# ssi-research/FQSS

Measured on AMD Instinct MI355X. Metric: QAT-step samples/sec + SI-SDR, ConvTasNet 2spk 8kHz W8A8, higher is better.
Workload: dtype f32; 1 GPU; ConvTasNet 2spk 8 kHz W8A8 QAT step (cfg 2), batch 8 x 4 s per GPU, quantizing phase; global_batch=8, segment_samples=32000, parallelism=dp1, optimizer=adam lr 1e-3 + clip 5.0

## Files before the change

### fqss_amd/csrc/qgemm.hip

```cpp
#include <type_traits>

#define FQSS_USES_GRAD_ADD
#include "fqss_dev.h"

namespace fqss {

typedef float f32x16 __attribute__((ext_vector_type(16)));
typedef __bf16 bf16x8 __attribute__((ext_vector_type(8)));
typedef short s16x4 __attribute__((ext_vector_type(4)));
typedef short s16x8 __attribute__((ext_vector_type(8)));

constexpr int QBM = 128, QBN = 64, QBK = 32;
constexpr int LDK = 40;
constexpr int LDN = 96;
constexpr int LDT = 36;
constexpr int WGRAD_BLOCKS = 256;

__device__ __forceinline__ unsigned short f2bf_trunc(float f) { return (unsigned short)(__float_as_uint(f) >> 16); }
__device__ __forceinline__ float bf_trunc(float f) { return __uint_as_float(__float_as_uint(f) & 0xFFFF0000u); }

__device__ __forceinline__ void split3(float g, unsigned short& b1, unsigned short& b2, unsigned short& b3) {
    const float h1 = bf_trunc(g);
    const float r1 = g - h1;
    const float h2 = bf_trunc(r1);
// ... 544 lines not shown
        for (int ks = 0; ks < W2_TK / 16; ++ks) {
            const int kk = ks * 16 + 8 * lh;
            const bf16x8 bfr = *reinterpret_cast<const bf16x8*>(&Bs[buf][wc * 32 + lr][kk]);
            bf16x8 af[GP];
#pragma unroll
            for (int p = 0; p < GP; ++p) af[p] = *reinterpret_cast<const bf16x8*>(&As[buf][p][wr * 32 + lr][kk]);
#pragma unroll
            for (int p = GP - 1; p >= 0; --p) acc = __builtin_amdgcn_mfma_f32_32x32x16_bf16(af[p], bfr, acc, 0, 0, 0);
        }
    };

    W2Stage st[W2_RING];
#pragma unroll
    for (int i = 0; i < W2_RING; ++i) load(st[i], i);
    w2_wait<3 * (W2_RING - 1)>(st[0]);
    convert_store(st[0], 0);
    load(st[0], W2_RING);
    __syncthreads();
    const bool first_half = wave < 4;
    for (int s = 0; s < nst; s += W2_RING) {
#pragma unroll
        for (int i = 0; i < W2_RING; ++i) {
            W2Stage& nx = st[(i + 1) % W2_RING];
            if (first_half) compute((s + i) & 1);
            w2_wait<3 * (W2_RING - 1)>(nx);
            convert_store(nx, s + i + 1);
            load(nx, s + i + 1 + W2_RING);
            if (!first_half) compute((s + i) & 1);
            __syncthreads();
        }
    }
#pragma unroll
    for (int i = 0; i < W2_RING; ++i) w2_wait<0>(st[i]);

#pragma unroll
    for (int i = 0; i < 2; ++i) {
        float v = rs_part[i];
#pragma unroll
        for (int o = 8; o > 0; o >>= 1) v += __shfl_xor(v, o, 64);
        if ((tid & 15) == 0) rsum[ar + 32 * i] = v;
    }
    __syncthreads();
    const float lo = *g.qmin_x, hi = *g.qmax_x;
    const float dx = (hi - lo) / 255.0f, mnx = lo;
#pragma unroll
    for (int r = 0; r < 16; ++r) {
        const int rl = (r & 3) + 8 * (r >> 2) + 4 * lh;
        const int row = row0 + wr * 32 + rl;
        const int col = col0 + wc * 32 + lr;
        if (row < g.M && col < g.N) grad_add(&g.C[(int64_t)row * g.ldc + col], dx * acc[r] + mnx * rsum[wr * 32 + rl]);
    }
}

constexpr int WGR_MAXJOBS = 25, WGR_TEAM = 8, WGR_TEAMS = 32, WGR_SLOT_FLOATS = W2_TM * 256;
struct WJob {
    const float* A; const float* A2; const unsigned char* Bc; float* C; const float* qmin; const float* qmax;
    int64_t lda, lda2, ldb, sAb, sA2b, sBb;
    int M, M1, N, K;
    int tiles_n, ntiles, spb, nstages;
    int ubeg, tile0;
    int wide;
};
struct WGroupArgs {
    int njobs, chunk, total, slots;
    unsigned* tickets; float* slabs;
    WJob j[WGR_MAXJOBS];
};
static_assert(sizeof(WGroupArgs) <= 4096, "the job table travels in the kernel arguments");
__device__ __forceinline__ void st16_sc1(float* p, const f32x4& v) {
#ifdef FQSS_NO_STORE_NOP
    asm volatile("global_store_dwordx4 %0, %1, off sc1" : : "v"(p), "v"(v) : "memory");
#else
    asm volatile("global_store_dwordx4 %0, %1, off sc1\n\ts_nop 1" : : "v"(p), "v"(v) : "memory");
#endif
}
__device__ __forceinline__ void ld16_sc1(f32x4& d, const float* p) { asm volatile("global_load_dwordx4 %0, %1, off sc1" : "=v"(d) : "v"(p) : "memory"); }

template <int GP, bool WIDE>
__device__ __forceinline__ void wgr_segment(const WGroupArgs& ga, const WJob& J, const int tile, const int s0, const int n, const int nparts,
                                            const int part, unsigned short* As_raw, unsigned short* Bs_raw, float* rsum, unsigned* ticket_s) {
    static_assert(GP == 3, "gz goes in three exact bf16 pieces");
    constexpr int TN = WIDE ? 256 : 128, NBF = WIDE ? 2 : 1;
    typedef unsigned short (*AsT)[GP][W2_TM][W2_LD];
    typedef unsigned short (*BsT)[TN][W2_LD];
    AsT As = reinterpret_cast<AsT>(As_raw);
    BsT Bs = reinterpret_cast<BsT>(Bs_raw);
    const int tid = threadIdx.x, lane = tid & 63;
    const int wave = __builtin_amdgcn_readfirstlane(tid >> 6);
    const int wr = wave >> 2, wc = wave & 3, lr = lane & 31, lh = lane >> 5;
    const int ar = tid >> 4, ac = (tid & 15) * 4;
    const int br = tid >> 2, bc = (tid & 3) * 16;
    const bool first_half = wave < 4;
    const int row0 = (tile / J.tiles_n) * W2_TM, col0 = (tile % J.tiles_n) * TN;
    const int K = J.K, spb = J.spb, nb = J.nstages / J.spb;
    const int ka_last = (K - 1) & ~3, kb_last = (K - 1) & ~15;
    const float* Arow[2];
    int64_t asb[2];
    bool aok[2];
#pragma unroll
    for (int i = 0; i < 2; ++i) {
        const int row = row0 + ar + 32 * i;
        aok[i] = row < J.M;
        const int rc = aok[i] ? row : 0;
        Arow[i] = (rc < J.M1) ? J.A + (int64_t)rc * J.lda : J.A2 + (int64_t)(rc - J.M1) * J.lda2;
        asb[i] = (rc < J.M1) ? J.sAb : J.sA2b;
    }
    const unsigned char* Brow[NBF];
#pragma unroll
    for (int f = 0; f < NBF; ++f) Brow[f] = J.Bc + (int64_t)min(col0 + br + 128 * f, J.N - 1) * J.ldb;
    const int64_t sBb = J.sBb;
    int lb = s0 / spb, lk = (s0 - lb * spb) * W2_TK;
    int ck = lk, cr = 0;
    const float* Ap[2] = {Arow[0] + lb * asb[0], Arow[1] + lb * asb[1]};
    int64_t boff = lb * sBb;
    struct Stage { f32x4 a[2]; u32x4 b[NBF]; };
    auto load = [&](Stage& st) {
#pragma unroll
        for (int i = 0; i < 2; ++i) wg_load16(st.a[i], Ap[i] + min(lk + ac, ka_last));
#pragma unroll
        for (int f = 0; f < NBF; ++f) wg_load16(st.b[f], Brow[f] + boff + min(lk + bc, kb_last));
        lk += W2_TK;
        if (lk >= spb * W2_TK) {
            lk = 0;
            lb = min(lb + 1, nb - 1);
            Ap[0] = Arow[0] + lb * asb[0];
            Ap[1] = Arow[1] + lb * asb[1];
            boff = lb * sBb;
        }
    };
    constexpr int NLD = 2 + NBF;
    auto wait_oldest = [&](Stage& st) {
        if constexpr (WIDE) asm volatile("s_waitcnt vmcnt(%4)" : "+v"(st.a[0]), "+v"(st.a[1]), "+v"(st.b[0]), "+v"(st.b[NBF - 1]) : "n"(NLD * (W2_RING - 1)) : "memory");
        else asm volatile("s_waitcnt vmcnt(%3)" : "+v"(st.a[0]), "+v"(st.a[1]), "+v"(st.b[0]) : "n"(NLD * (W2_RING - 1)) : "memory");
    };
    auto wait_all = [&](Stage& st) {
        if constexpr (WIDE) asm volatile("s_waitcnt vmcnt(0)" : "+v"(st.a[0]), "+v"(st.a[1]), "+v"(st.b[0]), "+v"(st.b[NBF - 1]) : : "memory");
        else asm volatile("s_waitcnt vmcnt(0)" : "+v"(st.a[0]), "+v"(st.a[1]), "+v"(st.b[0]) : : "memory");
    };
    float rs_part[2] = {0.f, 0.f};
    auto convert_store = [&](Stage& st, int buf) {
        const bool live = cr < n;
        const int k = ck + ac;
#pragma unroll
        for (int i = 0; i < 2; ++i) {
            float x[4];
#pragma unroll
            for (int e = 0; e < 4; ++e) x[e] = (aok[i] && live && k + e < K) ? st.a[i][e] : 0.0f;
            rs_part[i] += (x[0] + x[1]) + (x[2] + x[3]);
            uint32_t o1[2], o2[2], o3[2];
#pragma unroll
            for (int e = 0; e < 2; ++e) {
                const float a0 = x[2 * e], a1 = x[2 * e + 1];
                const float r0 = a0 - bf_trunc(a0), r1 = a1 - bf_trunc(a1);
                o1[e] = __builtin_amdgcn_perm(__float_as_uint(a1), __float_as_uint(a0), 0x07060302u);
                const float q0 = r0 - bf_trunc(r0), q1 = r1 - bf_trunc(r1);
                o2[e] = __builtin_amdgcn_perm(__float_as_uint(r1), __float_as_uint(r0), 0x07060302u);
                o3[e] = __builtin_amdgcn_perm(__float_as_uint(q1), __float_as_uint(q0), 0x07060302u);
            }
            const int row = ar + 32 * i;
            *reinterpret_cast<uint2*>(&As[buf][0][row][ac]) = make_uint2(o1[0], o1[1]);
            *reinterpret_cast<uint2*>(&As[buf][1][row][ac]) = make_uint2(o2[0], o2[1]);
            *reinterpret_cast<uint2*>(&As[buf][2][row][ac]) = make_uint2(o3[0], o3[1]);
        }
#pragma unroll
        for (int f = 0; f < NBF; ++f) {
            uint32_t o[8];
#pragma unroll
            for (int q = 0; q < 4; ++q) {
                const uint32_t w = st.b[f][q];
                const float f0 = (float)(w & 0xFFu), f1 = (float)((w >> 8) & 0xFFu);
                const float f2 = (float)((w >> 16) & 0xFFu), f3 = (float)(w >> 24);
                o[2 * q] = __builtin_amdgcn_perm(__float_as_uint(f1), __float_as_uint(f0), 0x07060302u);
                o[2 * q + 1] = __builtin_amdgcn_perm(__float_as_uint(f3), __float_as_uint(f2), 0x07060302u);
            }
            *reinterpret_cast<uint4*>(&Bs[buf][br + 128 * f][bc]) = make_uint4(o[0], o[1], o[2], o[3]);
            *reinterpret_cast<uint4*>(&Bs[buf][br + 128 * f][bc + 8]) = make_uint4(o[4], o[5], o[6], o[7]);
        }
        ++cr;
        ck += W2_TK;
        if (ck >= spb * W2_TK) ck = 0;
    };
    f32x16 acc[NBF];
#pragma unroll
    for (int f = 0; f < NBF; ++f)
#pragma unroll
        for (int r = 0; r < 16; ++r) acc[f][r] = 0.f;
    auto compute = [&](int buf) {
#pragma unroll
        for (int ks = 0; ks < W2_TK / 16; ++ks) {
            const int kk = ks * 16 + 8 * lh;
            bf16x8 bfr[NBF];
#pragma unroll
            for (int f = 0; f < NBF; ++f) bfr[f] = *reinterpret_cast<const bf16x8*>(&Bs[buf][wc * (32 * NBF) + 32 * f + lr][kk]);
            bf16x8 af[GP];
#pragma unroll
            for (int p = 0; p < GP; ++p) af[p] = *reinterpret_cast<const bf16x8*>(&As[buf][p][wr * 32 + lr][kk]);
#pragma unroll
            for (int p = GP - 1; p >= 0; --p)
#pragma unroll
                for (int f = 0; f < NBF; ++f) acc[f] = __builtin_amdgcn_mfma_f32_32x32x16_bf16(af[p], bfr[f], acc[f], 0, 0, 0);
        }
    };
    Stage st[W2_RING];
#pragma unroll
    for (int i = 0; i < W2_RING; ++i) load(st[i]);
    wait_oldest(st[0]);
    convert_store(st[0], 0);
    load(st[0]);
    __syncthreads();
    for (int s = 0; s < n; s += W2_RING) {
#pragma unroll
        for (int i = 0; i < W2_RING; ++i) {
            Stage& nx = st[(i + 1) % W2_RING];
            if (first_half) compute(i & 1);
            wait_oldest(nx);
            convert_store(nx, (i + 1) & 1);
            load(nx);
            if (!first_half) compute(i & 1);
            __syncthreads();
        }
    }
#pragma unroll
    for (int i = 0; i < W2_RING; ++i) wait_all(st[i]);
#pragma unroll
    for (int i = 0; i < 2; ++i) {
        float v = rs_part[i];
#pragma unroll
        for (int o = 8; o > 0; o >>= 1) v += __shfl_xor(v, o, 64);
        if ((tid & 15) == 0) rsum[ar + 32 * i] = v;
    }
    __syncthreads();
    const float lo = *J.qmin, hi = *J.qmax;
    const float dx = (hi - lo) / 255.0f, mnx = lo;
    constexpr int NV = 16 * NBF;
    float v[NV];
#pragma unroll
    for (int f = 0; f < NBF; ++f)
#pragma unroll
        for (int r = 0; r < 16; ++r) v[16 * f + r] = dx * acc[f][r] + mnx * rsum[wr * 32 + (r & 3) + 8 * (r >> 2) + 4 * lh];
    bool finish = nparts == 1;
    constexpr int SLOT = W2_TM * TN;
    if (!finish) {
        float* sl = ga.slabs + ((int64_t)(J.tile0 + tile) * ga.slots + part) * WGR_SLOT_FLOATS;
#pragma unroll
        for (int q = 0; q < NV / 4; ++q) st16_sc1(sl + ((int64_t)q * 512 + tid) * 4, f32x4{v[4 * q], v[4 * q + 1], v[4 * q + 2], v[4 * q + 3]});
        asm volatile("s_waitcnt vmcnt(0)" ::: "memory");
        __syncthreads();
        if (tid == 0) *ticket_s = __hip_atomic_fetch_add(&ga.tickets[J.tile0 + tile], 1u, __ATOMIC_RELAXED, __HIP_MEMORY_SCOPE_AGENT);
        __syncthreads();
        finish = *ticket_s == (unsigned)(nparts - 1);
        if (finish) {
            const float* s0p = ga.slabs + (int64_t)(J.tile0 + tile) * ga.slots * WGR_SLOT_FLOATS;
#pragma unroll
            for (int r = 0; r < NV; ++r) v[r] = 0.0f;
            for (int p = 0; p < nparts; ++p) {
#pragma unroll
                for (int h = 0; h < NBF; ++h) {
                    f32x4 t[4];
#pragma unroll
                    for (int q = 0; q < 4; ++q) ld16_sc1(t[q], s0p + (int64_t)p * WGR_SLOT_FLOATS + ((int64_t)(4 * h + q) * 512 + tid) * 4);
                    asm volatile("s_waitcnt vmcnt(0)" : "+v"(t[0]), "+v"(t[1]), "+v"(t[2]), "+v"(t[3]) : : "memory");
#pragma unroll
                    for (int q = 0; q < 4; ++q)
#pragma unroll
                        for (int e = 0; e < 4; ++e) v[16 * h + 4 * q + e] += t[q][e];
                }
            }
            if (tid == 0) __hip_atomic_store(&ga.tickets[J.tile0 + tile], 0u, __ATOMIC_RELAXED, __HIP_MEMORY_SCOPE_AGENT);
        }
    }
    static_assert(SLOT <= WGR_SLOT_FLOATS, "slab slots are sized for the wide tile");
    if (finish) {
        const int Mr = J.M, Nc = J.N;
        float* const Cp = J.C;
        float old[NV];
#pragma unroll
        for (int f = 0; f < NBF; ++f)
#pragma unroll
            for (int r = 0; r < 16; ++r) {
                const int row = row0 + wr * 32 + (r & 3) + 8 * (r >> 2) + 4 * lh, col = col0 + wc * (32 * NBF) + 32 * f + lr;
                old[16 * f + r] = (row < Mr && col < Nc) ? Cp[(int64_t)row * Nc + col] : 0.0f;
            }
#pragma unroll
        for (int f = 0; f < NBF; ++f)
#pragma unroll
            for (int r = 0; r < 16; ++r) {
                const int row = row0 + wr * 32 + (r & 3) + 8 * (r >> 2) + 4 * lh, col = col0 + wc * (32 * NBF) + 32 * f + lr;
                if (row < Mr && col < Nc) Cp[(int64_t)row * Nc + col] = old[16 * f + r] + v[16 * f + r];
            }
        asm volatile("s_waitcnt vmcnt(0)" ::: "memory");
    }
    __syncthreads();
}

template <int GP>
__global__ __launch_bounds__(512, 1) void k_qwgrad_group(WGroupArgs ga) {
    static_assert(GP == 3, "gz goes in three exact bf16 pieces");
    __shared__ __attribute__((aligned(16))) unsigned short As_raw[2 * GP * W2_TM * W2_LD];
    __shared__ __attribute__((aligned(16))) unsigned short Bs_raw[2 * 256 * W2_LD];
    __shared__ float rsum[W2_TM];
    __shared__ unsigned ticket_s;
    const int L = blockIdx.x, xcd = L % kXcds, slot = L / kXcds;
    const int team = (slot / WGR_TEAM) * kXcds + xcd, member = slot % WGR_TEAM;
    int u0 = team * ga.chunk;
    const int u1 = min(ga.total, u0 + ga.chunk);
    while (u0 < u1) {
        int jn = 0;
        for (int q = 1; q < ga.njobs; ++q) jn = (ga.j[q].ubeg <= u0) ? q : jn;
        const WJob& J = ga.j[jn];
        const int rel = u0 - J.ubeg, grp = rel / J.nstages, s0 = rel - grp * J.nstages;
        const int n = min(J.nstages - s0, u1 - u0);
        const int g0 = J.ubeg + grp * J.nstages;
        const int t_first = g0 / ga.chunk, nparts = (g0 + J.nstages - 1) / ga.chunk - t_first + 1, part = team - t_first;
        u0 += n;
        const int tile = grp * WGR_TEAM + member;
        if (tile >= J.ntiles) continue;
        if (J.wide) wgr_segment<GP, true>(ga, J, tile, s0, n, nparts, part, As_raw, Bs_raw, rsum, &ticket_s);
        else wgr_segment<GP, false>(ga, J, tile, s0, n, nparts, part, As_raw, Bs_raw, rsum, &ticket_s);
    }
}

__global__ __launch_bounds__(256) void k_wq_codes(const float* __restrict__ w, signed char* __restrict__ idx,
                                                   signed char* __restrict__ idxT, float* dw, float* rw, int Co, int Ci,
                                                   const float* __restrict__ qmin, const float* __restrict__ qmax, int n_bits) {
    __shared__ float red[4];
    const int co = blockIdx.x;
    const float L = wq_levels(n_bits), qlo = wq_qlo(n_bits), qhi = wq_qhi(n_bits);
    const float a = fmaxf(fabsf(qmin[co]), fabsf(qmax[co]));
    const float delta = (2.0f * a) / L;
    float s = 0.0f;
    for (int ci = threadIdx.x; ci < Ci; ci += 256) {
        const float X = rintf(w[(int64_t)co * Ci + ci] / delta);
        const float q = fminf(fmaxf(X, qlo), qhi);
        idx[(int64_t)co * Ci + ci] = (signed char)q;
        idxT[(int64_t)ci * Co + co] = (signed char)q;
        s += q;
    }
    float v[1] = {s};
    block_sum<float, 1>(v, red);
    if (threadIdx.x == 0) {
        dw[co] = delta;
        rw[co] = v[0];
    }
}

}

using namespace fqss;

extern "C" int fqss_wq_codes_bits(const float* w, int8_t* idx, int8_t* idxT, float* dw, float* rw, int Co, int Ci,
                                  const float* qmin, const float* qmax, int n_bits, fqss_stream_t stream) {
    FQSS_REQUIRE(w && idx && idxT && dw && rw && qmin && qmax && Co > 0 && Ci > 0, "bad args");
    FQSS_REQUIRE(n_bits >= FQSS_WQ_MIN_BITS && n_bits <= FQSS_WQ_MAX_BITS, "weight width outside 2..8 bits");
    hipLaunchKernelGGL(k_wq_codes, dim3((unsigned)Co), dim3(256), 0, (hipStream_t)stream, w, (signed char*)idx,
                       (signed char*)idxT, dw, rw, Co, Ci, qmin, qmax, n_bits);
    return launch_status("fqss_wq_codes_bits");
}

extern "C" int fqss_wq_codes(const float* w, int8_t* idx, int8_t* idxT, float* dw, float* rw, int Co, int Ci,
                             const float* qmin, const float* qmax, fqss_stream_t stream) {
    return fqss_wq_codes_bits(w, idx, idxT, dw, rw, Co, Ci, qmin, qmax, 8, stream);
}

struct QpwQuant {
    int act; const float* slope; const float *min1, *max1, *min2, *max2; uint8_t *yc1, *yc2; int64_t ld1, ld2;
    long long* stats;
    const FqssAddAfter *add1, *add2;
};

static int qpw_fwd_impl(const char* who, const uint8_t* xc, const int8_t* wi, const float* dw, const float* rw, const float* bias1,
                        const float* bias2, const float* qmin_x, const float* qmax_x, float* z1, float* z2, int B, int Ci, int Co1,
// ... 136 lines not shown

static int qpw_bwd_w_impl(const char* who, const float* gz1, const float* gz2, const uint8_t* xc, const float* qmin_x,
                          const float* qmax_x, float* gw, int B, int Ci, int Co1, int Co2, int M, int64_t ld_gz1, int64_t ld_gz2,
                          int64_t ld_xc, fqss_stream_t stream) {
    if (B == 0 || M == 0) return FQSS_OK;
    const int Co = Co1 + Co2;
    FQSS_REQUIRE(gz1 && xc && qmin_x && qmax_x && gw && (Co2 == 0 || gz2), "null tensor");
    FQSS_REQUIRE(B >= 0 && Ci > 0 && Co1 > 0 && Co2 >= 0 && M >= 0 && ld_gz1 >= M && ld_xc >= M, "bad shape");
    FQSS_REQUIRE(ld_gz1 % 4 == 0 && ld_xc % 16 == 0 && aligned16(gz1) && aligned16(xc) && ld_gz1 >= ((M + 3) & ~3),
                 "q-GEMM wgrad needs 16-B aligned gradient and code rows");
    FQSS_REQUIRE(Co2 == 0 || (ld_gz2 % 4 == 0 && aligned16(gz2) && ld_gz2 >= ((M + 3) & ~3)), "second gradient: 16-B aligned rows");
    if (B == 0 || M == 0) return FQSS_OK;
    QGemmArgs g{};
    g.A = gz1; g.B = xc; g.C = gw; g.M = Co; g.N = Ci; g.K = M;
    g.lda = ld_gz1; g.ldb = ld_xc; g.ldc = Ci;
    g.sAb = (int64_t)Co1 * ld_gz1; g.sBb = (int64_t)Ci * ld_xc; g.sCb = 0;
    g.M1 = Co1; g.A2 = gz2; g.lda2 = ld_gz2; g.sA2b = (int64_t)Co2 * ld_gz2; g.K1 = M;
    g.qmin_x = qmin_x; g.qmax_x = qmax_x;
    const int64_t tiles = cdiv(Co, 64) * cdiv(Ci, 128) * B;
    int want = (int)((WGRAD_BLOCKS + tiles / 2) / tiles);
    if (want < 1) want = 1;
    g.tiles_n = (int)cdiv(Ci, 128); g.tiles_m = (int)cdiv(Co, 64); g.batches = B;
    const int kchunk = (int)cdiv(cdiv(M, want), W2_RING * W2_TK) * W2_RING * W2_TK;
    g.kchunk = kchunk;
    g.ksplit = (int)cdiv(M, kchunk);
    hipLaunchKernelGGL(k_qwgrad2<3>, dim3(xcd_grid((int64_t)B * g.ksplit, (int64_t)g.tiles_m * g.tiles_n)), dim3(512), 0, (hipStream_t)stream, g);
    return launch_status(who);
}

extern "C" int fqss_qpw_bwd_w(const float* gz, const uint8_t* xc, const float* qmin_x, const float* qmax_x, float* gw,
                              int B, int Ci, int Co, int M, int64_t ld_gz, int64_t ld_xc, fqss_stream_t stream) {
    return qpw_bwd_w_impl("fqss_qpw_bwd_w", gz, nullptr, xc, qmin_x, qmax_x, gw, B, Ci, Co, 0, M, ld_gz, 0, ld_xc, stream);
}

extern "C" int fqss_qpw_bwd_w2(const float* gz1, const float* gz2, const uint8_t* xc, const float* qmin_x, const float* qmax_x,
                               float* gw, int B, int Ci, int Co1, int Co2, int M, int64_t ld_gz1, int64_t ld_gz2, int64_t ld_xc,
                               fqss_stream_t stream) {
    FQSS_REQUIRE(Co2 > 0, "second layer missing");
    return qpw_bwd_w_impl("fqss_qpw_bwd_w2", gz1, gz2, xc, qmin_x, qmax_x, gw, B, Ci, Co1, Co2, M, ld_gz1, ld_gz2, ld_xc, stream);
}

constexpr int64_t WGR_TICKET_BYTES = 65536;
static int wgr_plan(const FqssWgradJob* jobs, int n0, int n, WGroupArgs& ga, int64_t& slab_bytes) {
    int u = 0, t = 0, max_st = 0;
    ga.njobs = n;
    for (int q = 0; q < n; ++q) {
        const FqssWgradJob& f = jobs[n0 + q];
        WJob& J = ga.j[q];
        const int Co = f.Co1 + f.Co2;
        J.A = f.gz1; J.A2 = f.gz2; J.Bc = f.xc; J.C = f.gw; J.qmin = f.qmin_x; J.qmax = f.qmax_x;
        J.lda = f.ld_gz1; J.lda2 = f.ld_gz2; J.ldb = f.ld_xc;
        J.sAb = (int64_t)f.Co1 * f.ld_gz1; J.sA2b = (int64_t)f.Co2 * f.ld_gz2; J.sBb = (int64_t)f.Ci * f.ld_xc;
        J.M = Co; J.M1 = f.Co1; J.N = f.Ci; J.K = f.M;
        J.wide = f.Ci >= 256;
        J.tiles_n = (int)cdiv(f.Ci, J.wide ? 256 : W2_TN);
        J.ntiles = (int)cdiv(Co, W2_TM) * J.tiles_n;
        J.spb = (int)cdiv(f.M, W2_TK);
        J.nstages = f.B * J.spb;
        J.ubeg = u; J.tile0 = t;
        u += (int)cdiv(J.ntiles, WGR_TEAM) * J.nstages;
        t += J.ntiles;
        if (J.nstages > max_st) max_st = J.nstages;
    }
    ga.total = u;
    ga.chunk = (int)cdiv(u, WGR_TEAMS);
    ga.slots = (max_st - 1) / ga.chunk + 2;
    slab_bytes = (int64_t)t * ga.slots * WGR_SLOT_FLOATS * 4;
    return t;
}
static int wgr_check(const FqssWgradJob* jobs, int njobs) {
    FQSS_REQUIRE(jobs && njobs > 0, "no jobs");
    for (int q = 0; q < njobs; ++q) {
        const FqssWgradJob& f = jobs[q];
        FQSS_REQUIRE(f.gz1 && f.xc && f.qmin_x && f.qmax_x && f.gw && (f.Co2 == 0 || f.gz2), "null tensor");
        FQSS_REQUIRE(f.B > 0 && f.Ci > 0 && f.Co1 > 0 && f.Co2 >= 0 && f.M > 0 && f.ld_gz1 >= f.M && f.ld_xc >= f.M, "bad shape");
        FQSS_REQUIRE(f.ld_gz1 % 4 == 0 && f.ld_xc % 16 == 0 && aligned16(f.gz1) && aligned16(f.xc) && f.ld_gz1 >= ((f.M + 3) & ~3),
                     "q-GEMM wgrad needs 16-B aligned gradient and code rows");
        FQSS_REQUIRE(f.Co2 == 0 || (f.ld_gz2 % 4 == 0 && aligned16(f.gz2) && f.ld_gz2 >= ((f.M + 3) & ~3)), "second gradient: 16-B aligned rows");
        FQSS_REQUIRE((int64_t)f.B * cdiv(f.M, W2_TK) * cdiv(cdiv(f.Co1 + f.Co2, W2_TM) * cdiv(f.Ci, W2_TN), WGR_TEAM) < (1ll << 26), "job too large");
        for (int p = 0; p < q; ++p) FQSS_REQUIRE(jobs[p].gw != f.gw, "two jobs of one call accumulate into the same gw (plain read-modify-write)");
    }
    return FQSS_OK;
}

extern "C" int64_t fqss_qpw_bwd_w_group_ws(const FqssWgradJob* jobs, int njobs) {
    if (wgr_check(jobs, njobs) != FQSS_OK) return -1;
    int64_t need = 0;
    const int per = (int)cdiv(njobs, cdiv(njobs, WGR_MAXJOBS));
    for (int n0 = 0; n0 < njobs; n0 += per) {
        WGroupArgs ga{};
        int64_t sb = 0;
        const int t = wgr_plan(jobs, n0, njobs - n0 < per ? njobs - n0 : per, ga, sb);
        if ((int64_t)t * 4 > WGR_TICKET_BYTES) { set_error("fqss_qpw_bwd_w_group_ws: more than 16384 tiles in one launch"); return -1; }
        if (sb > need) need = sb;
    }
    return WGR_TICKET_BYTES + need;
}

extern "C" int fqss_qpw_bwd_w_group(const FqssWgradJob* jobs, int njobs, void* ws, int64_t ws_bytes, fqss_stream_t stream) {
    if (njobs == 0) return FQSS_OK;
    if (int rc = wgr_check(jobs, njobs)) return rc;
    FQSS_REQUIRE(ws && aligned16(ws), "workspace: 16-B aligned device memory (fqss_qpw_bwd_w_group_ws bytes, zero-filled when first used)");
    const int per = (int)cdiv(njobs, cdiv(njobs, WGR_MAXJOBS));
    for (int n0 = 0; n0 < njobs; n0 += per) {
        WGroupArgs ga{};
        int64_t sb = 0;
        const int t = wgr_plan(jobs, n0, njobs - n0 < per ? njobs - n0 : per, ga, sb);
        FQSS_REQUIRE((int64_t)t * 4 <= WGR_TICKET_BYTES && WGR_TICKET_BYTES + sb <= ws_bytes, "workspace too small (fqss_qpw_bwd_w_group_ws)");
        ga.tickets = (unsigned*)ws;
        ga.slabs = (float*)((char*)ws + WGR_TICKET_BYTES);
        hipLaunchKernelGGL(k_qwgrad_group<3>, dim3(WGR_TEAMS * WGR_TEAM), dim3(512), 0, (hipStream_t)stream, ga);
        if (int rc = launch_status("fqss_qpw_bwd_w_group")) return rc;
    }
    return FQSS_OK;
}

static int pwconv_fwd_x3_impl(const char* who, bool six, const float* x, const float* w, const float* bias, float* z, int B, int Ci, int Co,
                              int M, int64_t ld_x, int64_t ld_z, fqss_stream_t stream) {
    if (B == 0 || M == 0) return FQSS_OK;
    FQSS_REQUIRE(x && w && z, "null tensor");
    FQSS_REQUIRE(B >= 0 && Ci > 0 && Co > 0 && M >= 0 && ld_x >= M && ld_z >= M, "bad shape");
    FQSS_REQUIRE(Ci % 4 == 0 && ld_x % 4 == 0 && aligned16(x) && aligned16(w) && ld_x >= ((M + 3) & ~3),
                 "x3 GEMM needs Ci % 4 == 0 and 16-B aligned activation rows");
    FQSS_REQUIRE(aligned16(z) && ld_z % 4 == 0, "output rows must be 16-B aligned");
    if (B == 0 || M == 0) return FQSS_OK;
    QGemmArgs g{};
    g.A = w; g.B = x; g.C = z; g.M = Co; g.N = M; g.K = Ci;
    g.lda = Ci; g.ldb = ld_x; g.ldc = ld_z;
    g.sAb = 0; g.sBb = (int64_t)Ci * ld_x; g.sCb = (int64_t)Co * ld_z;
    g.bias = bias; g.ksplit = 1; g.kchunk = Ci; g.M1 = Co; g.K1 = Ci;
    g.tiles_n = (int)cdiv(M, QBN); g.tiles_m = (int)cdiv(Co, QBM); g.batches = B;
    if (six) hipLaunchKernelGGL((k_qgemm<3, 2>), dim3(xcd_grid((int64_t)g.tiles_n * B, g.tiles_m)), dim3(256), 0, (hipStream_t)stream, g);
    else hipLaunchKernelGGL((k_qgemm<3>), dim3(xcd_grid((int64_t)g.tiles_n * B, g.tiles_m)), dim3(256), 0, (hipStream_t)stream, g);
    return launch_status(who);
}

extern "C" int fqss_pwconv_fwd_wq(const float* x, const int8_t* wi, const float* dw, const float* bias, float* z, int B, int Ci, int Co, int M,
                                  int64_t ld_x, int64_t ld_z, fqss_stream_t stream) {
    if (B == 0 || M == 0) return FQSS_OK;
    FQSS_REQUIRE(x && wi && dw && z, "null tensor");
    FQSS_REQUIRE(B >= 0 && Ci >= 16 && Co > 0 && M >= 0 && ld_x >= M && ld_z >= M, "bad shape");
    FQSS_REQUIRE(Ci % 16 == 0 && ld_x % 4 == 0 && aligned16(x) && aligned16(wi) && ld_x >= ((M + 3) & ~3),
                 "coded-weight forward needs Ci % 16 == 0 and 16-B aligned activation rows");
    FQSS_REQUIRE(aligned16(z) && ld_z % 4 == 0, "output rows must be 16-B aligned");
    QGemmArgs g{};
    g.A = wi; g.B = x; g.C = z; g.M = Co; g.N = M; g.K = Ci;
    g.lda = Ci; g.ldb = ld_x; g.ldc = ld_z;
    g.sAb = 0; g.sBb = (int64_t)Ci * ld_x; g.sCb = (int64_t)Co * ld_z;
    g.dw = dw; g.bias = bias; g.ksplit = 1; g.kchunk = Ci; g.M1 = Co; g.K1 = Ci;
    g.B2 = x; g.ldb2 = ld_x; g.sB2b = g.sBb;
    g.tiles_n = (int)cdiv(M, QBN); g.tiles_m = (int)cdiv(Co, QBM); g.batches = B;
    hipLaunchKernelGGL((k_qgemm<4>), dim3(xcd_grid((int64_t)g.tiles_n * B, g.tiles_m)), dim3(256), 0, (hipStream_t)stream, g);
    return launch_status("fqss_pwconv_fwd_wq");
}

static int conv2_impl(const char* who, int mode, const void* A, const float* Bsig, const float* dw, const float* bias, float* C, int B, int Cr, int M,
                      int taps, int kw, int base, int row_step, int col_step, int64_t N, int64_t plane_in, int64_t plane_out,
                      fqss_stream_t stream) {
    if (B == 0 || N == 0) return FQSS_OK;
    FQSS_REQUIRE(A && Bsig && C && (mode == 3 || dw), "null tensor");
    FQSS_REQUIRE(B > 0 && Cr > 0 && M > 0 && taps >= 1 && kw >= 1 && taps % kw == 0 && N > 0 && plane_out >= N, "bad shape");
    const int64_t K = (int64_t)Cr * taps;
    FQSS_REQUIRE(K < (1 << 16), "reduction too long for the reciprocal division of the implicit loader");
    FQSS_REQUIRE(mode == 3 ? (K % 4 == 0) : (K % 16 == 0), "implicit convolution: (channels x taps) % 16 == 0 for coded weights, % 4 == 0 for float ones");
// ... 55 lines not shown
```

Baseline: 631.3 samples/s.

## Restructure grouped q-wgrad kernel: gradient fragments in registers, 256-thread blocks, 128x128 tiles

The grouped weight-gradient kernel drops the LDS staging of the three-way bf16 split of the gradient. Each wave now loads its own 32 gradient rows straight into registers and splits them into MFMA fragments. Blocks shrink from 512 to 256 threads with two blocks per CU, and each covers a fixed 128x128 tile, replacing the wide/narrow variants. Team sizes change to 4 members by 128 teams, and the code-operand conversion is pipelined one stage ahead. The intent is to cut LDS traffic and the barrier-driven convert step and to raise occupancy, at the cost of much higher register pressure (64 accumulators plus 8 f32x4 loads per stage in a 2-deep ring).

```diff
diff --git a/fqss_amd/csrc/qgemm.hip b/fqss_amd/csrc/qgemm.hip
--- a/fqss_amd/csrc/qgemm.hip
+++ b/fqss_amd/csrc/qgemm.hip
@@ -620,14 +620,13 @@
     }
 }
 
-constexpr int WGR_MAXJOBS = 25, WGR_TEAM = 8, WGR_TEAMS = 32, WGR_SLOT_FLOATS = W2_TM * 256;
+constexpr int WGR_MAXJOBS = 25, WGR_TEAM = 4, WGR_TEAMS = 128, WGR_TM = 128, WGR_TN = 128, WGR_RING = 2, WGR_SLOT_FLOATS = WGR_TM * WGR_TN;
 struct WJob {
     const float* A; const float* A2; const unsigned char* Bc; float* C; const float* qmin; const float* qmax;
     int64_t lda, lda2, ldb, sAb, sA2b, sBb;
     int M, M1, N, K;
     int tiles_n, ntiles, spb, nstages;
     int ubeg, tile0;
-    int wide;
 };
 struct WGroupArgs {
     int njobs, chunk, total, slots;
@@ -643,175 +642,185 @@
 #endif
 }
 __device__ __forceinline__ void ld16_sc1(f32x4& d, const float* p) { asm volatile("global_load_dwordx4 %0, %1, off sc1" : "=v"(d) : "v"(p) : "memory"); }
-
-template <int GP, bool WIDE>
+template <int OFF>
+__device__ __forceinline__ void wg_load16_at(f32x4& d, const void* p) {
+    asm volatile("global_load_dwordx4 %0, %1, off offset:%2" : "=v"(d) : "v"(p), "n"(OFF) : "memory");
+}
+
+struct WgrStage {
+    f32x4 a[8];
+    u32x4 b[2];
+};
+constexpr int WGR_NLD = 10;
+template <int N>
+__device__ __forceinline__ void wgr_wait(WgrStage& st) {
+    asm volatile("s_waitcnt vmcnt(%10)"
+                 : "+v"(st.a[0]), "+v"(st.a[1]), "+v"(st.a[2]), "+v"(st.a[3]), "+v"(st.a[4]), "+v"(st.a[5]), "+v"(st.a[6]), "+v"(st.a[7]),
+                   "+v"(st.b[0]), "+v"(st.b[1])
+                 : "n"(N) : "memory");
+}
+
+template <int GP>
 __device__ __forceinline__ void wgr_segment(const WGroupArgs& ga, const WJob& J, const int tile, const int s0, const int n, const int nparts,
-                                            const int part, unsigned short* As_raw, unsigned short* Bs_raw, float* rsum, unsigned* ticket_s) {
+                                            const int part, unsigned short* Bs_raw, float* rsum, unsigned* ticket_s) {
     static_assert(GP == 3, "gz goes in three exact bf16 pieces");
-    constexpr int TN = WIDE ? 256 : 128, NBF = WIDE ? 2 : 1;
-    typedef unsigned short (*AsT)[GP][W2_TM][W2_LD];
-    typedef unsigned short (*BsT)[TN][W2_LD];
-    AsT As = reinterpret_cast<AsT>(As_raw);
+    typedef unsigned short (*BsT)[WGR_TN][W2_LD];
     BsT Bs = reinterpret_cast<BsT>(Bs_raw);
     const int tid = threadIdx.x, lane = tid & 63;
     const int wave = __builtin_amdgcn_readfirstlane(tid >> 6);
-    const int wr = wave >> 2, wc = wave & 3, lr = lane & 31, lh = lane >> 5;
-    const int ar = tid >> 4, ac = (tid & 15) * 4;
+    const int lr = lane & 31, lh = lane >> 5, ao = 8 * lh;
     const int br = tid >> 2, bc = (tid & 3) * 16;
-    const bool first_half = wave < 4;
-    const int row0 = (tile / J.tiles_n) * W2_TM, col0 = (tile % J.tiles_n) * TN;
+    const int row0 = (tile / J.tiles_n) * WGR_TM, col0 = (tile % J.tiles_n) * WGR_TN;
     const int K = J.K, spb = J.spb, nb = J.nstages / J.spb;
     const int ka_last = (K - 1) & ~3, kb_last = (K - 1) & ~15;
-    const float* Arow[2];
-    int64_t asb[2];
-    bool aok[2];
-#pragma unroll
-    for (int i = 0; i < 2; ++i) {
-        const int row = row0 + ar + 32 * i;
-        aok[i] = row < J.M;
-        const int rc = aok[i] ? row : 0;
-        Arow[i] = (rc < J.M1) ? J.A + (int64_t)rc * J.lda : J.A2 + (int64_t)(rc - J.M1) * J.lda2;
-        asb[i] = (rc < J.M1) ? J.sAb : J.sA2b;
-    }
-    const unsigned char* Brow[NBF];
-#pragma unroll
-    for (int f = 0; f < NBF; ++f) Brow[f] = J.Bc + (int64_t)min(col0 + br + 128 * f, J.N - 1) * J.ldb;
+    const int row = row0 + wave * 32 + lr;
+    const int rc = row < J.M ? row : 0;
+    const bool second = rc >= J.M1;
+    const float* const Arow = second ? J.A2 + (int64_t)(rc - J.M1) * J.lda2 : J.A + (int64_t)rc * J.lda;
+    const int64_t asb = second ? J.sA2b : J.sAb;
+    const unsigned char* Brow[2];
+#pragma unroll
+    for (int f = 0; f < 2; ++f) Brow[f] = J.Bc + (int64_t)min(col0 + br + 64 * f, J.N - 1) * J.ldb;
     const int64_t sBb = J.sBb;
-    int lb = s0 / spb, lk = (s0 - lb * spb) * W2_TK;
-    int ck = lk, cr = 0;
-    const float* Ap[2] = {Arow[0] + lb * asb[0], Arow[1] + lb * asb[1]};
-    int64_t boff = lb * sBb;
-    struct Stage { f32x4 a[2]; u32x4 b[NBF]; };
-    auto load = [&](Stage& st) {
-#pragma unroll
-        for (int i = 0; i < 2; ++i) wg_load16(st.a[i], Ap[i] + min(lk + ac, ka_last));
-#pragma unroll
-        for (int f = 0; f < NBF; ++f) wg_load16(st.b[f], Brow[f] + boff + min(lk + bc, kb_last));
-        lk += W2_TK;
-        if (lk >= spb * W2_TK) {
-            lk = 0;
-            lb = min(lb + 1, nb - 1);
-            Ap[0] = Arow[0] + lb * asb[0];
-            Ap[1] = Arow[1] + lb * asb[1];
-            boff = lb * sBb;
-        }
-    };
-    constexpr int NLD = 2 + NBF;
-    auto wait_oldest = [&](Stage& st) {
-        if constexpr (WIDE) asm volatile("s_waitcnt vmcnt(%4)" : "+v"(st.a[0]), "+v"(st.a[1]), "+v"(st.b[0]), "+v"(st.b[NBF - 1]) : "n"(NLD * (W2_RING - 1)) : "memory");
-        else asm volatile("s_waitcnt vmcnt(%3)" : "+v"(st.a[0]), "+v"(st.a[1]), "+v"(st.b[0]) : "n"(NLD * (W2_RING - 1)) : "memory");
-    };
-    auto wait_all = [&](Stage& st) {
-        if constexpr (WIDE) asm volatile("s_waitcnt vmcnt(0)" : "+v"(st.a[0]), "+v"(st.a[1]), "+v"(st.b[0]), "+v"(st.b[NBF - 1]) : : "memory");
-        else asm volatile("s_waitcnt vmcnt(0)" : "+v"(st.a[0]), "+v"(st.a[1]), "+v"(st.b[0]) : : "memory");
-    };
-    float rs_part[2] = {0.f, 0.f};
-    auto convert_store = [&](Stage& st, int buf) {
-        const bool live = cr < n;
-        const int k = ck + ac;
-#pragma unroll
-        for (int i = 0; i < 2; ++i) {
-            float x[4];
-#pragma unroll
-            for (int e = 0; e < 4; ++e) x[e] = (aok[i] && live && k + e < K) ? st.a[i][e] : 0.0f;
-            rs_part[i] += (x[0] + x[1]) + (x[2] + x[3]);
-            uint32_t o1[2], o2[2], o3[2];
-#pragma unroll
-            for (int e = 0; e < 2; ++e) {
-                const float a0 = x[2 * e], a1 = x[2 * e + 1];
-                const float r0 = a0 - bf_trunc(a0), r1 = a1 - bf_trunc(a1);
-                o1[e] = __builtin_amdgcn_perm(__float_as_uint(a1), __float_as_uint(a0), 0x07060302u);
-                const float q0 = r0 - bf_trunc(r0), q1 = r1 - bf_trunc(r1);
-                o2[e] = __builtin_amdgcn_perm(__float_as_uint(r1), __float_as_uint(r0), 0x07060302u);
-                o3[e] = __builtin_amdgcn_perm(__float_as_uint(q1), __float_as_uint(q0), 0x07060302u);
-            }
-            const int row = ar + 32 * i;
-            *reinterpret_cast<uint2*>(&As[buf][0][row][ac]) = make_uint2(o1[0], o1[1]);
-            *reinterpret_cast<uint2*>(&As[buf][1][row][ac]) = make_uint2(o2[0], o2[1]);
-            *reinterpret_cast<uint2*>(&As[buf][2][row][ac]) = make_uint2(o3[0], o3[1]);
-        }
-#pragma unroll
-        for (int f = 0; f < NBF; ++f) {
+    int gb = s0 / spb, gk = (s0 - gb * spb) * W2_TK;
+    int qb = gb, qk = gk;
+    int pk = gk;
+    auto advance = [&](int& b, int& k) {
+        k += W2_TK;
+        if (k >= spb * W2_TK) { k = 0; b = min(b + 1, nb - 1); }
+    };
+    auto load_codes = [&](u32x4 (&b)[2]) {
+        const int64_t off = qb * sBb + min(qk + bc, kb_last);
+#pragma unroll
+        for (int f = 0; f < 2; ++f) wg_load16(b[f], Brow[f] + off);
+        advance(qb, qk);
+    };
+    auto load_gz = [&](f32x4 (&a)[8]) {
+        const float* const p = Arow + gb * asb;
+        if (gk + W2_TK <= K) {
+            const float* const q = p + gk + ao;
+            wg_load16_at<0>(a[0], q);   wg_load16_at<16>(a[1], q);
+            wg_load16_at<64>(a[2], q);  wg_load16_at<80>(a[3], q);
+            wg_load16_at<128>(a[4], q); wg_load16_at<144>(a[5], q);
+            wg_load16_at<192>(a[6], q); wg_load16_at<208>(a[7], q);
+        } else {
+#pragma unroll
+            for (int j = 0; j < 8; ++j) wg_load16(a[j], p + min(gk + (j >> 1) * 16 + ao + 4 * (j & 1), ka_last));
+        }
+        advance(gb, gk);
+    };
+    auto load = [&](WgrStage& st) {
+        load_gz(st.a);
+        load_codes(st.b);
+    };
+    auto convert = [&](const u32x4 (&b)[2], int buf) {
+#pragma unroll
+        for (int f = 0; f < 2; ++f) {
             uint32_t o[8];
 #pragma unroll
             for (int q = 0; q < 4; ++q) {
-                const uint32_t w = st.b[f][q];
+                const uint32_t w = b[f][q];
                 const float f0 = (float)(w & 0xFFu), f1 = (float)((w >> 8) & 0xFFu);
                 const float f2 = (float)((w >> 16) & 0xFFu), f3 = (float)(w >> 24);
                 o[2 * q] = __builtin_amdgcn_perm(__float_as_uint(f1), __float_as_uint(f0), 0x07060302u);
                 o[2 * q + 1] = __builtin_amdgcn_perm(__float_as_uint(f3), __float_as_uint(f2), 0x07060302u);
             }
-            *reinterpret_cast<uint4*>(&Bs[buf][br + 128 * f][bc]) = make_uint4(o[0], o[1], o[2], o[3]);
-            *reinterpret_cast<uint4*>(&Bs[buf][br + 128 * f][bc + 8]) = make_uint4(o[4], o[5], o[6], o[7]);
-        }
-        ++cr;
-        ck += W2_TK;
-        if (ck >= spb * W2_TK) ck = 0;
-    };
-    f32x16 acc[NBF];
-#pragma unroll
-    for (int f = 0; f < NBF; ++f)
+            *reinterpret_cast<uint4*>(&Bs[buf][br + 64 * f][bc]) = make_uint4(o[0], o[1], o[2], o[3]);
+            *reinterpret_cast<uint4*>(&Bs[buf][br + 64 * f][bc + 8]) = make_uint4(o[4], o[5], o[6], o[7]);
+        }
+    };
+    float rs_part = 0.f;
+    f32x16 acc[4];
+#pragma unroll
+    for (int f = 0; f < 4; ++f)
 #pragma unroll
         for (int r = 0; r < 16; ++r) acc[f][r] = 0.f;
-    auto compute = [&](int buf) {
+    auto mask = [&](WgrStage& st, int kmax) {
+#pragma unroll
+        for (int j = 0; j < 8; ++j) {
+            const int k = pk + (j >> 1) * 16 + ao + 4 * (j & 1);
+#pragma unroll
+            for (int e = 0; e < 4; ++e) st.a[j][e] = (k + e < kmax) ? st.a[j][e] : 0.0f;
+        }
+    };
+    auto split = [&](const WgrStage& st, int ks, bf16x8 (&af)[GP]) {
+        float x[8];
+#pragma unroll
+        for (int e = 0; e < 8; ++e) x[e] = st.a[2 * ks + (e >> 2)][e & 3];
+        rs_part += ((x[0] + x[1]) + (x[2] + x[3])) + ((x[4] + x[5]) + (x[6] + x[7]));
+        u32x4 o1, o2, o3;
+#pragma unroll
+        for (int e = 0; e < 4; ++e) {
+            const float a0 = x[2 * e], a1 = x[2 * e + 1];
+            const float r0 = a0 - bf_trunc(a0), r1 = a1 - bf_trunc(a1);
+            o1[e] = __builtin_amdgcn_perm(__float_as_uint(a1), __float_as_uint(a0), 0x07060302u);
+            const float q0 = r0 - bf_trunc(r0), q1 = r1 - bf_trunc(r1);
+            o2[e] = __builtin_amdgcn_perm(__float_as_uint(r1), __float_as_uint(r0), 0x07060302u);
+            o3[e] = __builtin_amdgcn_perm(__float_as_uint(q1), __float_as_uint(q0), 0x07060302u);
+        }
+        af[0] = __builtin_bit_cast(bf16x8, o1);
+        af[1] = __builtin_bit_cast(bf16x8, o2);
+        af[2] = __builtin_bit_cast(bf16x8, o3);
+    };
+    auto compute = [&](const WgrStage& st, int buf) {
+        bf16x8 af[2][GP];
+        split(st, 0, af[0]);
 #pragma unroll
         for (int ks = 0; ks < W2_TK / 16; ++ks) {
-            const int kk = ks * 16 + 8 * lh;
-            bf16x8 bfr[NBF];
-#pragma unroll
-            for (int f = 0; f < NBF; ++f) bfr[f] = *reinterpret_cast<const bf16x8*>(&Bs[buf][wc * (32 * NBF) + 32 * f + lr][kk]);
-            bf16x8 af[GP];
-#pragma unroll
-            for (int p = 0; p < GP; ++p) af[p] = *reinterpret_cast<const bf16x8*>(&As[buf][p][wr * 32 + lr][kk]);
+            bf16x8 bfr[4];
+#pragma unroll
+            for (int f = 0; f < 4; ++f) bfr[f] = *reinterpret_cast<const bf16x8*>(&Bs[buf][32 * f + lr][ks * 16 + ao]);
+            if (ks + 1 < W2_TK / 16) split(st, ks + 1, af[(ks + 1) & 1]);
 #pragma unroll
             for (int p = GP - 1; p >= 0; --p)
 #pragma unroll
-                for (int f = 0; f < NBF; ++f) acc[f] = __builtin_amdgcn_mfma_f32_32x32x16_bf16(af[p], bfr[f], acc[f], 0, 0, 0);
-        }
-    };
-    Stage st[W2_RING];
-#pragma unroll
-    for (int i = 0; i < W2_RING; ++i) load(st[i]);
-    wait_oldest(st[0]);
-    convert_store(st[0], 0);
-    load(st[0]);
+                for (int f = 0; f < 4; ++f) acc[f] = __builtin_amdgcn_mfma_f32_32x32x16_bf16(af[ks & 1][p], bfr[f], acc[f], 0, 0, 0);
+        }
+    };
+    WgrStage st[WGR_RING];
+    {
+        u32x4 b0[2];
+        load_codes(b0);
+#pragma unroll
+        for (int i = 0; i < WGR_RING; ++i) load(st[i]);
+        asm volatile("s_waitcnt vmcnt(%2)" : "+v"(b0[0]), "+v"(b0[1]) : "n"(WGR_NLD * WGR_RING) : "memory");
+        convert(b0, 0);
+    }
     __syncthreads();
-    for (int s = 0; s < n; s += W2_RING) {
-#pragma unroll
-        for (int i = 0; i < W2_RING; ++i) {
-            Stage& nx = st[(i + 1) % W2_RING];
-            if (first_half) compute(i & 1);
-            wait_oldest(nx);
-            convert_store(nx, (i + 1) & 1);
-            load(nx);
-            if (!first_half) compute(i & 1);
+    for (int s = 0; s < n; s += WGR_RING) {
+#pragma unroll
+        for (int i = 0; i < WGR_RING; ++i) {
+            WgrStage& cur = st[i];
+            const int buf = (s + i) & 1;
+            wgr_wait<WGR_NLD * (WGR_RING - 1)>(cur);
+            convert(cur.b, buf ^ 1);
+            const int kmax = s + i < n ? K : 0;
+            if (pk + W2_TK > kmax) mask(cur, kmax);
+            compute(cur, buf);
+            pk += W2_TK;
+            if (pk >= spb * W2_TK) pk = 0;
+            load(cur);
             __syncthreads();
         }
     }
 #pragma unroll
-    for (int i = 0; i < W2_RING; ++i) wait_all(st[i]);
-#pragma unroll
-    for (int i = 0; i < 2; ++i) {
-        float v = rs_part[i];
-#pragma unroll
-        for (int o = 8; o > 0; o >>= 1) v += __shfl_xor(v, o, 64);
-        if ((tid & 15) == 0) rsum[ar + 32 * i] = v;
-    }
+    for (int i = 0; i < WGR_RING; ++i) wgr_wait<0>(st[i]);
+    rs_part += __shfl_xor(rs_part, 32, 64);
+    if (lh == 0) rsum[wave * 32 + lr] = rs_part;
     __syncthreads();
     const float lo = *J.qmin, hi = *J.qmax;
     const float dx = (hi - lo) / 255.0f, mnx = lo;
-    constexpr int NV = 16 * NBF;
+    constexpr int NV = 64;
     float v[NV];
 #pragma unroll
-    for (int f = 0; f < NBF; ++f)
-#pragma unroll
-        for (int r = 0; r < 16; ++r) v[16 * f + r] = dx * acc[f][r] + mnx * rsum[wr * 32 + (r & 3) + 8 * (r >> 2) + 4 * lh];
+    for (int f = 0; f < 4; ++f)
+#pragma unroll
+        for (int r = 0; r < 16; ++r) v[16 * f + r] = dx * acc[f][r] + mnx * rsum[wave * 32 + (r & 3) + 8 * (r >> 2) + 4 * lh];
     bool finish = nparts == 1;
-    constexpr int SLOT = W2_TM * TN;
     if (!finish) {
         float* sl = ga.slabs + ((int64_t)(J.tile0 + tile) * ga.slots + part) * WGR_SLOT_FLOATS;
 #pragma unroll
-        for (int q = 0; q < NV / 4; ++q) st16_sc1(sl + ((int64_t)q * 512 + tid) * 4, f32x4{v[4 * q], v[4 * q + 1], v[4 * q + 2], v[4 * q + 3]});
+        for (int q = 0; q < NV / 4; ++q) st16_sc1(sl + ((int64_t)q * 256 + tid) * 4, f32x4{v[4 * q], v[4 * q + 1], v[4 * q + 2], v[4 * q + 3]});
         asm volatile("s_waitcnt vmcnt(0)" ::: "memory");
         __syncthreads();
         if (tid == 0) *ticket_s = __hip_atomic_fetch_add(&ga.tickets[J.tile0 + tile], 1u, __ATOMIC_RELAXED, __HIP_MEMORY_SCOPE_AGENT);
@@ -823,10 +832,10 @@
             for (int r = 0; r < NV; ++r) v[r] = 0.0f;
             for (int p = 0; p < nparts; ++p) {
 #pragma unroll
-                for (int h = 0; h < NBF; ++h) {
+                for (int h = 0; h < NV / 16; ++h) {
                     f32x4 t[4];
 #pragma unroll
-                    for (int q = 0; q < 4; ++q) ld16_sc1(t[q], s0p + (int64_t)p * WGR_SLOT_FLOATS + ((int64_t)(4 * h + q) * 512 + tid) * 4);
+                    for (int q = 0; q < 4; ++q) ld16_sc1(t[q], s0p + (int64_t)p * WGR_SLOT_FLOATS + ((int64_t)(4 * h + q) * 256 + tid) * 4);
                     asm volatile("s_waitcnt vmcnt(0)" : "+v"(t[0]), "+v"(t[1]), "+v"(t[2]), "+v"(t[3]) : : "memory");
 #pragma unroll
                     for (int q = 0; q < 4; ++q)
@@ -837,36 +846,33 @@
             if (tid == 0) __hip_atomic_store(&ga.tickets[J.tile0 + tile], 0u, __ATOMIC_RELAXED, __HIP_MEMORY_SCOPE_AGENT);
         }
     }
-    static_assert(SLOT <= WGR_SLOT_FLOATS, "slab slots are sized for the wide tile");
     if (finish) {
         const int Mr = J.M, Nc = J.N;
         float* const Cp = J.C;
-        float old[NV];
-#pragma unroll
-        for (int f = 0; f < NBF; ++f)
+#pragma unroll
+        for (int f = 0; f < 4; ++f) {
+            float old[16];
 #pragma unroll
             for (int r = 0; r < 16; ++r) {
-                const int row = row0 + wr * 32 + (r & 3) + 8 * (r >> 2) + 4 * lh, col = col0 + wc * (32 * NBF) + 32 * f + lr;
-                old[16 * f + r] = (row < Mr && col < Nc) ? Cp[(int64_t)row * Nc + col] : 0.0f;
-            }
-#pragma unroll
-        for (int f = 0; f < NBF; ++f)
+                const int orow = row0 + wave * 32 + (r & 3) + 8 * (r >> 2) + 4 * lh, col = col0 + 32 * f + lr;
+                old[r] = (orow < Mr && col < Nc) ? Cp[(int64_t)orow * Nc + col] : 0.0f;
+            }
 #pragma unroll
             for (int r = 0; r < 16; ++r) {
-                const int row = row0 + wr * 32 + (r & 3) + 8 * (r >> 2) + 4 * lh, col = col0 + wc * (32 * NBF) + 32 * f + lr;
-                if (row < Mr && col < Nc) Cp[(int64_t)row * Nc + col] = old[16 * f + r] + v[16 * f + r];
-            }
+                const int orow = row0 + wave * 32 + (r & 3) + 8 * (r >> 2) + 4 * lh, col = col0 + 32 * f + lr;
+                if (orow < Mr && col < Nc) Cp[(int64_t)orow * Nc + col] = old[r] + v[16 * f + r];
+            }
+        }
         asm volatile("s_waitcnt vmcnt(0)" ::: "memory");
     }
     __syncthreads();
 }
 
 template <int GP>
-__global__ __launch_bounds__(512, 1) void k_qwgrad_group(WGroupArgs ga) {
+__global__ __launch_bounds__(256, 2) void k_qwgrad_group(WGroupArgs ga) {
     static_assert(GP == 3, "gz goes in three exact bf16 pieces");
-    __shared__ __attribute__((aligned(16))) unsigned short As_raw[2 * GP * W2_TM * W2_LD];
-    __shared__ __attribute__((aligned(16))) unsigned short Bs_raw[2 * 256 * W2_LD];
-    __shared__ float rsum[W2_TM];
+    __shared__ __attribute__((aligned(16))) unsigned short Bs_raw[2 * WGR_TN * W2_LD];
+    __shared__ float rsum[WGR_TM];
     __shared__ unsigned ticket_s;
     const int L = blockIdx.x, xcd = L % kXcds, slot = L / kXcds;
     const int team = (slot / WGR_TEAM) * kXcds + xcd, member = slot % WGR_TEAM;
@@ -883,8 +889,7 @@
         u0 += n;
         const int tile = grp * WGR_TEAM + member;
         if (tile >= J.ntiles) continue;
-        if (J.wide) wgr_segment<GP, true>(ga, J, tile, s0, n, nparts, part, As_raw, Bs_raw, rsum, &ticket_s);
-        else wgr_segment<GP, false>(ga, J, tile, s0, n, nparts, part, As_raw, Bs_raw, rsum, &ticket_s);
+        wgr_segment<GP>(ga, J, tile, s0, n, nparts, part, Bs_raw, rsum, &ticket_s);
     }
 }
 
@@ -1127,9 +1132,8 @@
         J.lda = f.ld_gz1; J.lda2 = f.ld_gz2; J.ldb = f.ld_xc;
         J.sAb = (int64_t)f.Co1 * f.ld_gz1; J.sA2b = (int64_t)f.Co2 * f.ld_gz2; J.sBb = (int64_t)f.Ci * f.ld_xc;
         J.M = Co; J.M1 = f.Co1; J.N = f.Ci; J.K = f.M;
-        J.wide = f.Ci >= 256;
-        J.tiles_n = (int)cdiv(f.Ci, J.wide ? 256 : W2_TN);
-        J.ntiles = (int)cdiv(Co, W2_TM) * J.tiles_n;
+        J.tiles_n = (int)cdiv(f.Ci, WGR_TN);
+        J.ntiles = (int)cdiv(Co, WGR_TM) * J.tiles_n;
         J.spb = (int)cdiv(f.M, W2_TK);
         J.nstages = f.B * J.spb;
         J.ubeg = u; J.tile0 = t;
@@ -1152,7 +1156,7 @@
         FQSS_REQUIRE(f.ld_gz1 % 4 == 0 && f.ld_xc % 16 == 0 && aligned16(f.gz1) && aligned16(f.xc) && f.ld_gz1 >= ((f.M + 3) & ~3),
                      "q-GEMM wgrad needs 16-B aligned gradient and code rows");
         FQSS_REQUIRE(f.Co2 == 0 || (f.ld_gz2 % 4 == 0 && aligned16(f.gz2) && f.ld_gz2 >= ((f.M + 3) & ~3)), "second gradient: 16-B aligned rows");
-        FQSS_REQUIRE((int64_t)f.B * cdiv(f.M, W2_TK) * cdiv(cdiv(f.Co1 + f.Co2, W2_TM) * cdiv(f.Ci, W2_TN), WGR_TEAM) < (1ll << 26), "job too large");
+        FQSS_REQUIRE((int64_t)f.B * cdiv(f.M, W2_TK) * cdiv(cdiv(f.Co1 + f.Co2, WGR_TM) * cdiv(f.Ci, WGR_TN), WGR_TEAM) < (1ll << 26), "job too large");
         for (int p = 0; p < q; ++p) FQSS_REQUIRE(jobs[p].gw != f.gw, "two jobs of one call accumulate into the same gw (plain read-modify-write)");
     }
     return FQSS_OK;
@@ -1184,7 +1188,7 @@
         FQSS_REQUIRE((int64_t)t * 4 <= WGR_TICKET_BYTES && WGR_TICKET_BYTES + sb <= ws_bytes, "workspace too small (fqss_qpw_bwd_w_group_ws)");
         ga.tickets = (unsigned*)ws;
         ga.slabs = (float*)((char*)ws + WGR_TICKET_BYTES);
-        hipLaunchKernelGGL(k_qwgrad_group<3>, dim3(WGR_TEAMS * WGR_TEAM), dim3(512), 0, (hipStream_t)stream, ga);
+        hipLaunchKernelGGL(k_qwgrad_group<3>, dim3(WGR_TEAMS * WGR_TEAM), dim3(256), 0, (hipStream_t)stream, ga);
         if (int rc = launch_status("fqss_qpw_bwd_w_group")) return rc;
     }
     return FQSS_OK;
```

Result: no change. 634.7 samples/s, median of 6 (+0.5%).
